# norlab-ulaval/norlab_icp_mapper

Hardware: AMD Instinct MI355X
Metric: ICP iterations/sec, 100k-pt scan vs 1M-pt map (higher is better)
Workload: dtype f32; 1 GPU; single synthetic 100000-pt scan vs 1000000-pt map, point-to-point ICP, KDTreeMatcher knn 1 maxDist 2.0 epsilon 0, TrimmedDist 0.85, fixed 20 iterations per registration; chain=p2p, scene=box+pillars sigma=0.01 seeds 42/43/44 (SURVEY.md 8d), parallelism=scan-sharded x1, map replicated

## Files before the change

### norlab_icp_mapper_amd/csrc/common.h

```cpp
#pragma once

#include <hip/hip_runtime.h>
#include <stdint.h>
#include <math.h>
#include <cstring>
#include <string>
#include <vector>
#include <unordered_map>
#include <mutex>
#include <map>
#include <cstdlib>
#include <shared_mutex>

#include "../../include/icpmi.h"

#define ICPMI_NV 32
#define ICPMI_MAX_OUTLIER 8
#define ICPMI_MAX_SMOOTH 16
#define ICPMI_SEL_BINS 2048
#ifndef ICPMI_S2_COPIES
#define ICPMI_S2_COPIES 8
#endif
#define ICPMI_S2_C0 4096
#define ICPMI_S2_F0 (ICPMI_S2_C0 + ICPMI_S2_COPIES * 256)
#ifndef ICPMI_S2_FCOPIES
#define ICPMI_S2_FCOPIES 1
#endif
#define ICPMI_S2_C1 (ICPMI_S2_F0 + ICPMI_S2_FCOPIES * 65536)
#define ICPMI_S2_F1 (ICPMI_S2_C1 + 256)
#define ICPMI_ACC_COPIES 2
#define ICPMI_ACC_MAX_ADDS 128
#define ICPMI_ACC_PAD 16
#define ICPMI_ACC_U64 (ICPMI_ACC_COPIES * ICPMI_NV * 2 * ICPMI_ACC_PAD)
#define ICPMI_ACC_IDX(copy, i, limb) ((((copy) * ICPMI_NV + (i)) * 2 + (limb)) * ICPMI_ACC_PAD)
#define ICPMI_ACC_FLAG (ICPMI_ACC_IDX(0, 0, 0) + 8)
#define ICPMI_S2_ACC (ICPMI_S2_F1 + 65536)
#define ICPMI_WIN_BINS 7
#ifndef ICPMI_WIN_COPIES
#define ICPMI_WIN_COPIES 8
#endif
#define ICPMI_WIN_PAD 16
#define ICPMI_WIN_HDR (ICPMI_WIN_COPIES * 3 * ICPMI_WIN_PAD)
#define ICPMI_WIN_U64 (ICPMI_WIN_HDR + ICPMI_WIN_PAD)
#define ICPMI_WIN_MAX_COUNT (1ll << 21)
#define ICPMI_S2_WIN (ICPMI_S2_ACC + 2 * ICPMI_ACC_U64)
#define ICPMI_SELHIST_WORDS (ICPMI_S2_WIN + 2 * ICPMI_WIN_U64)
#define ICPMI_S2_FIDX(b) ((((b) & 255u) << 8) | ((b) >> 8))

#define ICPMI_MAX_K 32

#ifdef __HIPCC__
typedef float icpmi_vf4 __attribute__((ext_vector_type(4)));
#ifdef ICPMI_NT_STREAMS
__device__ __forceinline__ float4 ld_stream(const float4* p) { const icpmi_vf4 v = __builtin_nontemporal_load(reinterpret_cast<const icpmi_vf4*>(p)); return make_float4(v.x, v.y, v.z, v.w); }
__device__ __forceinline__ float ld_stream(const float* p) { return __builtin_nontemporal_load(p); }
__device__ __forceinline__ int ld_stream(const int* p) { return __builtin_nontemporal_load(p); }
__device__ __forceinline__ void st_stream(float4* p, float4 v) { icpmi_vf4 w; w.x = v.x; w.y = v.y; w.z = v.z; w.w = v.w; __builtin_nontemporal_store(w, reinterpret_cast<icpmi_vf4*>(p)); }
__device__ __forceinline__ void st_stream(float* p, float v) { __builtin_nontemporal_store(v, p); }
__device__ __forceinline__ void st_stream(int* p, int v) { __builtin_nontemporal_store(v, p); }
#else
template <class T> __device__ __forceinline__ T ld_stream(const T* p) { return *p; }
template <class T> __device__ __forceinline__ void st_stream(T* p, T v) { *p = v; }
#endif

struct WaveRun { bool head; int rank; int len; int head_lane; };
__device__ __forceinline__ WaveRun wave_run(unsigned key, bool valid)
{
    const int lane = threadIdx.x & 63;
    const unsigned prev = (unsigned)__shfl_up((int)key, 1, 64);
    const bool pvalid = __shfl_up((int)valid, 1, 64) != 0;
    const bool head = valid && (lane == 0 || !pvalid || prev != key);
    const unsigned long long heads = __ballot(head);
    const unsigned long long valids = __ballot(valid);
    WaveRun r;
    r.head = head;
    const unsigned long long below = heads & ((lane == 63) ? ~0ull : ((2ull << lane) - 1ull));
    r.head_lane = below ? 63 - __clzll((long long)below) : lane;
    r.rank = lane - r.head_lane;
// ... 747 lines not shown
```

### norlab_icp_mapper_amd/csrc/loop.hip

```cpp
#include "common.h"
#include "solve.h"
#include <cstring>

namespace {

template <int PASS, int MODE = 0>
__global__ __launch_bounds__(256) void sel_hist_kernel(const float* __restrict__ d2, int64_t count,
                                                       const IcpState* __restrict__ st, unsigned* __restrict__ ghist, int nb_scale = 0)
{
    if (st->done) return;
    if (blockIdx.x == 0 && threadIdx.x == 0) nn_stamp_close(const_cast<IcpState*>(st));
    if (MODE != 0 && nb_scale != 0 && st->iter + 1 > nb_scale) return;
    if (MODE == 3 && st->iter != 0) return;
    __shared__ unsigned h[ICPMI_SEL_BINS];
    for (int b = threadIdx.x; b < ICPMI_SEL_BINS; b += 256) h[b] = 0;
    __syncthreads();
    const unsigned prefix = st->sel_prefix;
    const float med = MODE == 2 ? st->robust_med : 0.f;
    for (int64_t i = (int64_t)blockIdx.x * 256 + threadIdx.x; i < count; i += (int64_t)gridDim.x * 256) {
        float v = d2[i];
        if (MODE == 0 || MODE == 3) { if (!(v != INFINITY && v > 0.f)) continue; }
        else {
            if (v == INFINITY) continue;
            if (MODE == 2) v = fabsf(v - med);
// ... 505 lines not shown
                const float rz = fmaf(T[10], az, fmaf(T[6], ay, T[2] * ax));
                ax = rx; ay = ry; az = rz;
            }
            const float4 b = ref_normals[sidx];
            const float dot = fmaf(az, b.z, fmaf(ay, b.y, ax * b.x));
            w *= (dot > cosf(prm)) ? 1.f : 0.f;
        } else if (EXT && type == ICPMI_OUT_GENERICDESCRIPTOR) {
            const int ip = lc.out_iparam[f];
            const float v = (ip & ICPMI_GEN_SOURCE_READING) ? lc.read_scalar[qi] : ref_scalar[orig];
            w *= (ip & ICPMI_GEN_SOFT) ? v : ((ip & ICPMI_GEN_LARGER) ? (v > prm ? 1.f : 0.f) : (v < prm ? 1.f : 0.f));
        } else if (EXT && type == ICPMI_OUT_ROBUST) {
            const int ip = lc.out_iparam[f];
            const int se = (ip >> 4) & 15, fct = ip & 15;
            const float sc = se != ICPMI_SCALE_NONE ? st->robust_scale : 1.f;
            const float res = ((ip >> 8) & 15) == ICPMI_DIST_POINT2PLANE ? plane2 : d2;
            const float kk = se != ICPMI_SCALE_BERG ? prm : (fct == ICPMI_ROB_CAUCHY ? 4.3040f : fct == ICPMI_ROB_TUKEY ? 7.0589f : fct == ICPMI_ROB_HUBER ? 2.0138f : prm);
            const float e2 = res / (sc * sc);
            const float apx = lc.out_param3[f];
            float rw = robust_weight(fct, e2, kk);
            if (apx > 0.f && apx != INFINITY && e2 >= apx * apx) rw = 0.f;
            w *= rw;
        }
    }
    return w;
}

__host__ __device__ __forceinline__ int acc_threads(int k) { return k > 1 ? 1024 : 256; }
__host__ __device__ __forceinline__ int acc_blocks_dev(int64_t count, int cap, int bt = 256)
{
    const int64_t nb = (count + bt - 1) / bt;
    return (int)(nb < 1 ? 1 : (nb > cap ? cap : nb));
}

template <int MIN, bool FUSED, bool EXT, int BT = 256>
__global__ __launch_bounds__(BT) void accumulate_kernel(const float4* __restrict__ reading, BatchArgs ba, int acc_cap, LoopCfg lc,
                                                         IcpState* __restrict__ st, const float4* __restrict__ map,
                                                         const float4* __restrict__ normals,
                                                         const float4* __restrict__ read_normals,
                                                         const int* __restrict__ sidx, const float* __restrict__ d2a,
                                                         unsigned* __restrict__ hists,
                                                         int fused_slot, int is_median, float factor,
                                                         const float4* __restrict__ match_pt, const int* __restrict__ qindex,
                                                         const float* __restrict__ ref_scalar, const float4* __restrict__ pnm)
{
    const int n = ba.n[blockIdx.y];
    const int nbe = acc_blocks_dev((int64_t)n * lc.k, acc_cap, BT);
    if ((int)blockIdx.x >= nbe) return;
    {
        const size_t qo = (size_t)blockIdx.y * (size_t)ba.qstride;
        reading += qo; sidx += qo * lc.k; d2a += qo * lc.k;
        if (match_pt) match_pt += qo;
        if (qindex) qindex += qo;
        if (read_normals) read_normals += qo;
        hists += (size_t)blockIdx.y * ICPMI_SELHIST_WORDS;
        st += blockIdx.y;
    }
    const int64_t count = (int64_t)n * lc.k;
    const int64_t stride = (int64_t)nbe * BT;
    const int64_t gtid = (int64_t)blockIdx.x * BT + threadIdx.x;
#ifdef ICPMI_ACC_STRIDED
    const int64_t estep = stride;
    const int64_t e_first = gtid, e_end = count;
#else
    const int64_t estep = BT;
    const int wgc = (nbe & 7) == 0 ? (int)(blockIdx.x & 7) * (nbe >> 3) + (int)(blockIdx.x >> 3) : (int)blockIdx.x;
    const int64_t per_wg = (count + nbe - 1) / nbe;
    const int64_t e_first = (int64_t)wgc * per_wg + threadIdx.x;
    const int64_t e_end = ((int64_t)wgc + 1) * per_wg < count ? ((int64_t)wgc + 1) * per_wg : count;
#endif
    constexpr int PF = BT > 256 ? 3 : 2;
    float pd2[PF]; int ps[PF]; float4 pr[PF], pq[PF];
#pragma unroll
    for (int u = 0; u < PF; ++u) {
        const int64_t e = e_first + u * estep;
        const bool in = e < e_end;
        pd2[u] = in ? ld_stream(d2a + e) : INFINITY;
        ps[u] = in ? ld_stream(sidx + e) : -1;
        pr[u] = ld_stream(reading + (in ? (int)(e / lc.k) : 0));
        pq[u] = (match_pt && in) ? ld_stream(match_pt + e) : ((pnm && ps[u] >= 0) ? pnm[2 * (size_t)ps[u]] : make_float4(0.f, 0.f, 0.f, 0.f));
    }
    const unsigned cv = (FUSED && threadIdx.x < 256) ? hists[ICPMI_S2_C1 + threadIdx.x] : 0u;
    float4 pn[PF];
#pragma unroll
    for (int u = 0; u < PF; ++u)
        pn[u] = (MIN == ICPMI_MIN_POINT_TO_PLANE && ps[u] >= 0) ? (pnm ? pnm[2 * (size_t)ps[u] + 1] : normals[ps[u]]) : make_float4(0.f, 0.f, 0.f, 0.f);
    if (st->done) return;
    if (blockIdx.x == 0 && threadIdx.x == 0) nn_stamp_close(const_cast<IcpState*>(st));
    float fused_limit = 0.f;
    if (FUSED) {
        __shared__ unsigned shsel[16];
        unsigned bin, rem, total;
        block_find_rank_2tier<1>(cv, hists + ICPMI_S2_F1, false, 0.f, st->sel_rank_l[0], shsel, bin, rem, total);
        const float q = __uint_as_float((st->sel_prefix_l[0] << 16) | bin);
        fused_limit = is_median ? factor * q : q;
        if (blockIdx.x == 0 && threadIdx.x == 0) st->limits[fused_slot] = fused_limit;
        for (int64_t i = gtid; i < ICPMI_S2_COPIES * 256 + ICPMI_S2_FCOPIES * 65536; i += stride) hists[ICPMI_S2_C0 + i] = 0;
        if (lc.k > 1) for (int64_t i = gtid; i < 2 * ICPMI_WIN_U64; i += stride) hists[ICPMI_S2_WIN + i] = 0;
    }
    constexpr int NVAL = MIN == ICPMI_MIN_POINT_TO_PLANE ? 27 : (MIN == ICPMI_MIN_POINT_TO_POINT ? 16 : 0);
    double acc[NVAL > 0 ? NVAL : 1];
#pragma unroll
    for (int i = 0; i < (NVAL > 0 ? NVAL : 1); ++i) acc[i] = 0.0;
    double wsum = 0.0, cnt = 0.0;
    double b2d[3] = {0.0, 0.0, 0.0};
    const float* T = st->T_iter;
    auto pair = [&](int64_t e, float d2, int s, float4 r, float4 qkept, float4 nkept, bool have_n) {
        if (d2 == INFINITY) return;
        const int qi = (int)(e / lc.k);
        float w;
        if (EXT) {
            const float3 pe = xf_point(T, r.x, r.y, r.z, r.w);
            const float4 qe = (match_pt || (pnm && have_n)) ? qkept : (pnm ? pnm[2 * (size_t)s] : map[s]);
            float plane2 = 0.f;
            if (normals) {
                const float4 ne = have_n && MIN == ICPMI_MIN_POINT_TO_PLANE ? nkept : (pnm ? pnm[2 * (size_t)s + 1] : normals[s]);
                const float dx = pe.x - qe.x, dy = pe.y - qe.y, dz = pe.z - qe.z;
                const float dot = dx * ne.x + dy * ne.y + dz * ne.z;
                plane2 = dot * dot;
            }
            w = match_weight<true>(lc, st, d2, T, read_normals, qindex ? qindex[qi] : qi, normals, s, FUSED ? fused_slot : -1, fused_limit,
                                   ref_scalar, __float_as_int(qe.w), plane2);
        } else w = match_weight(lc, st, d2, T, read_normals, qindex ? qindex[qi] : qi, normals, s, FUSED ? fused_slot : -1, fused_limit);
        if (w == 0.f) return;
        wsum += w; cnt += 1.0;
        if (MIN == ICPMI_MIN_IDENTITY) return;
        const float3 p = xf_point(T, r.x, r.y, r.z, r.w);
        const float4 q = (match_pt || (pnm && have_n)) ? qkept : (pnm ? pnm[2 * (size_t)s] : map[s]);
        if (MIN == ICPMI_MIN_POINT_TO_POINT) {
// ... 27 lines not shown
            }
        }
    };
#pragma unroll
    for (int u = 0; u < PF; ++u) pair(e_first + u * estep, pd2[u], ps[u], pr[u], pq[u], pn[u], true);
    for (int64_t e = e_first + PF * estep; e < e_end; e += estep)
        pair(e, d2a[e], sidx[e], reading[(int)(e / lc.k)], match_pt ? match_pt[e] : make_float4(0.f, 0.f, 0.f, 0.f),
             make_float4(0.f, 0.f, 0.f, 0.f), false);
    __shared__ double sh[BT / 64][ICPMI_NV];
    const int lane = threadIdx.x & 63, wv = threadIdx.x >> 6;
    double val[ICPMI_NV];
#pragma unroll
    for (int i = 0; i < ICPMI_NV; ++i) val[i] = i < NVAL ? acc[i < NVAL ? i : 0] : 0.0;
    val[27] = wsum; val[28] = cnt;
    if (EXT) { val[29] = b2d[0]; val[30] = b2d[1]; val[31] = b2d[2]; }
#pragma unroll
    for (int s = 0; s < 5; ++s) {
        const int m = 1 << s;
        const int nkeep = 16 >> s;
        const bool upper = (lane & m) != 0;
#pragma unroll
        for (int i = 0; i < nkeep; ++i) {
            const double send = upper ? val[i] : val[i + nkeep];
            const double keep = upper ? val[i + nkeep] : val[i];
            val[i] = keep + __shfl_xor(send, m, 64);
        }
    }
    val[0] += __shfl_xor(val[0], 32, 64);
    if (lane < 32) {
        const int idx = ((lane & 1) << 4) | ((lane & 2) << 2) | (lane & 4) | ((lane & 8) >> 2) | ((lane & 16) >> 4);
        sh[wv][idx] = val[0];
    }
    __syncthreads();
    if (threadIdx.x < ICPMI_NV) {
        const int i = threadIdx.x;
        double v = 0.0;
        if (i < NVAL || i == 27 || i == 28 || (EXT && i > 28)) {
            v = sh[0][i] + sh[1][i] + sh[2][i] + sh[3][i];
#pragma unroll
            for (int w2 = 4; w2 < BT / 64; ++w2) v += sh[w2][i];
        }
        unsigned long long* acc = reinterpret_cast<unsigned long long*>(hists + ICPMI_S2_ACC);
        if (v != 0.0) {
            if (!(fabs(v) < 0x1p77)) atomicOr(reinterpret_cast<unsigned*>(acc + ICPMI_ACC_FLAG), 1u);
            else {
                const double hi = rint(v * 0x1p-16);
                const double lo = v - hi * 65536.0;
                const long long H = (long long)hi, Lq = __double2ll_rn(lo * 0x1p40);
                const int cp = blockIdx.x & (ICPMI_ACC_COPIES - 1);
                if (H) atomicAdd(acc + ICPMI_ACC_IDX(cp, i, 0), (unsigned long long)H);
                if (Lq) atomicAdd(acc + ICPMI_ACC_IDX(cp, i, 1), (unsigned long long)Lq);
            }
        }
    }
}

__device__ __forceinline__ void mirror_state(const IcpState* st, IcpState* mirror)
{
    const unsigned* src = reinterpret_cast<const unsigned*>(st);
    unsigned* dst = reinterpret_cast<unsigned*>(mirror);
    constexpr int W = (int)(sizeof(IcpState) / sizeof(unsigned));
    for (int i = threadIdx.x; i < W; i += 64) dst[i] = __hip_atomic_load(src + i, __ATOMIC_RELAXED, __HIP_MEMORY_SCOPE_AGENT);
}

__global__ __launch_bounds__(256) void solve_kernel(IcpState* __restrict__ st, unsigned* __restrict__ hists, int clear, LoopCfg lc,
                                                    float* __restrict__ T_step_out, double* __restrict__ sums_out, unsigned* __restrict__ progress,
                                                    IcpState* __restrict__ mirror)
{
    st += blockIdx.x;
    unsigned long long* acc = reinterpret_cast<unsigned long long*>(hists + (size_t)blockIdx.x * ICPMI_SELHIST_WORDS + ICPMI_S2_ACC);
    if (progress) progress += blockIdx.x;
    if (threadIdx.x == 0 && st->hard_count) { st->hard_total += st->hard_count; st->hard_count = 0; }
    if (st->done) {
        if (mirror && threadIdx.x < 64) mirror_state(st, mirror + blockIdx.x);
        if (threadIdx.x == 0) publish_progress(st, progress);
        return;
    }
    solve_body(st, acc, clear != 0, lc, T_step_out, sums_out);
    if (threadIdx.x == 0 && st->done) st->t_done = (unsigned long long)wall_clock64();
    if (mirror) {
        __syncthreads();
        if (threadIdx.x < 64 && __hip_atomic_load(&st->done, __ATOMIC_RELAXED, __HIP_MEMORY_SCOPE_AGENT)) mirror_state(st, mirror + blockIdx.x);
    }
    if (threadIdx.x == 0) publish_progress(st, progress);
}

__global__ __launch_bounds__(256) void centre_kernel(BatchSrc src, BatchArgs ba, float mx, float my, float mz, float4* __restrict__ out)
{
    const int64_t n = ba.n[blockIdx.y];
    const float4* __restrict__ scan = src.p[blockIdx.y];
    out += (size_t)blockIdx.y * (size_t)ba.qstride;
    const int64_t i = (int64_t)blockIdx.x * 256 + threadIdx.x;
    if (i >= n) return;
    const float4 p = scan[i];
    out[i] = make_float4(fmaf(-mx, p.w, p.x), fmaf(-my, p.w, p.y), fmaf(-mz, p.w, p.z), p.w);
// ... 506 lines not shown
    }
    if (slot >= 0) {
        const float quant = lc.out_type[slot] == ICPMI_OUT_MEDIANDIST ? 0.5f : lc.out_param[slot];
        const BatchArgs ba = cur_batch(c, count / lc.k);
        if (!c->nn_builds_hist0)
        {
            int hb0 = (int)std::min<int64_t>((count + 4095) / 4096, 256);
            if (hb0 < 1) hb0 = 1;
            hipLaunchKernelGGL(sel2_hist0_kernel, dim3(hb0, ba.nscan), dim3(256), 0, c->stream, c->d_d2, ba, lc.k, c->d_state, c->d_selhist, quant,
                               c->nn_builds_win ? 1 : 0);
        }
        int hb2 = (int)std::min<int64_t>((count + 511) / 512, 512);
        if (hb2 < 1) hb2 = 1;
        hipLaunchKernelGGL(sel2_scan_hist_kernel, dim3(hb2, ba.nscan), dim3(256), 0, c->stream, c->d_d2, ba, lc.k, c->d_state, c->d_selhist, quant,
                           (c->nn_builds_win && !c->nn_builds_hist0) ? 1 : 0);
        return;
    }
    for (int f = 0; f < lc.n_out; ++f) {
        const int type = lc.out_type[f];
        if (type != ICPMI_OUT_TRIMMEDDIST && type != ICPMI_OUT_MEDIANDIST) continue;
        const int is_med = type == ICPMI_OUT_MEDIANDIST;
        const float quant = is_med ? 0.5f : lc.out_param[f];
        const float factor = lc.out_param[f];
        hipLaunchKernelGGL((sel_hist_kernel<0, 0>), dim3(hb), dim3(256), 0, c->stream, c->d_d2, count, c->d_state, c->d_selhist, 0);
        hipLaunchKernelGGL(sel_scan_kernel<0>, dim3(1), dim3(256), 0, c->stream, c->d_state, c->d_selhist, quant, f, is_med, factor, 0, 0);
        hipLaunchKernelGGL((sel_hist_kernel<1, 0>), dim3(hb), dim3(256), 0, c->stream, c->d_d2, count, c->d_state, c->d_selhist, 0);
        hipLaunchKernelGGL(sel_scan_kernel<1>, dim3(1), dim3(256), 0, c->stream, c->d_state, c->d_selhist, quant, f, is_med, factor, 0, 0);
        hipLaunchKernelGGL((sel_hist_kernel<2, 0>), dim3(hb), dim3(256), 0, c->stream, c->d_d2, count, c->d_state, c->d_selhist, 0);
        hipLaunchKernelGGL(sel_scan_kernel<2>, dim3(1), dim3(256), 0, c->stream, c->d_state, c->d_selhist, quant, f, is_med, factor, 0, 0);
    }
}

template <int MIN, bool FUSED, bool EXT>
static void launch_accumulate_ext(icpmi_ctx* c, int64_t n, const LoopCfg& lc, int nb, int slot);

template <int MIN, bool FUSED>
static void launch_accumulate(icpmi_ctx* c, int64_t n, const LoopCfg& lc, int nb, int slot)
{
    if (lc.ext) launch_accumulate_ext<MIN, FUSED, true>(c, n, lc, nb, slot);
    else launch_accumulate_ext<MIN, FUSED, false>(c, n, lc, nb, slot);
}

template <int MIN, bool FUSED, bool EXT>
static void launch_accumulate_ext(icpmi_ctx* c, int64_t n, const LoopCfg& lc, int nb, int slot)
{
    const float4* rn = lc.has_read_normals ? c->d_read_normals : nullptr;
    const int is_med = slot >= 0 && lc.out_type[slot] == ICPMI_OUT_MEDIANDIST;
    const float factor = slot >= 0 ? lc.out_param[slot] : 0.f;
    const bool sorted = c->nn_out_sorted;
    const BatchArgs ba = cur_batch(c, n);
    if (lc.k > 1) {
        hipLaunchKernelGGL((accumulate_kernel<MIN, FUSED, EXT, 1024>), dim3(nb, ba.nscan), dim3(1024), 0, c->stream, sorted ? c->d_qsorted : c->d_reading, ba, acc_cap(), lc, c->d_state,
                           c->d_map_sorted, c->has_normals ? c->d_normals_sorted : (const float4*)nullptr, rn, c->d_sidx, c->d_d2, c->d_selhist, slot, is_med, factor,
                           (const float4*)nullptr, sorted ? c->d_qindex : (const int*)nullptr, (EXT && c->raw_has_scalar) ? c->d_raw_s : (const float*)nullptr,
                           (MIN == ICPMI_MIN_POINT_TO_PLANE && c->has_normals && c->d_map_pn) ? c->d_map_pn : (const float4*)nullptr);
        return;
    }
    hipLaunchKernelGGL((accumulate_kernel<MIN, FUSED, EXT>), dim3(nb, ba.nscan), dim3(256), 0, c->stream, sorted ? c->d_qsorted : c->d_reading, ba, acc_cap(), lc, c->d_state,
                       c->d_map_sorted, c->has_normals ? c->d_normals_sorted : (const float4*)nullptr, rn, c->d_sidx, c->d_d2, c->d_selhist, slot, is_med, factor,
                       (sorted && lc.k == 1) ? c->d_match_pt : (const float4*)nullptr, sorted ? c->d_qindex : (const int*)nullptr,
                       (EXT && c->raw_has_scalar) ? c->d_raw_s : (const float*)nullptr,
                       (lc.k > 1 && MIN == ICPMI_MIN_POINT_TO_PLANE && c->has_normals && c->d_map_pn) ? c->d_map_pn : (const float4*)nullptr);
}

static void enqueue_accumulate_solve(icpmi_ctx* c, int64_t n, const LoopCfg& lc, float* d_Tstep, double* d_sums)
{
    const int64_t count = n * lc.k;
    const int nb = acc_blocks(count, acc_threads(lc.k));
    const int slot = fused_filter_slot(lc);
    const bool fused = slot >= 0;
    if (lc.minimizer == ICPMI_MIN_POINT_TO_PLANE) {
        if (fused) launch_accumulate<ICPMI_MIN_POINT_TO_PLANE, true>(c, n, lc, nb, slot);
        else launch_accumulate<ICPMI_MIN_POINT_TO_PLANE, false>(c, n, lc, nb, slot);
    } else if (lc.minimizer == ICPMI_MIN_POINT_TO_POINT) {
        if (fused) launch_accumulate<ICPMI_MIN_POINT_TO_POINT, true>(c, n, lc, nb, slot);
        else launch_accumulate<ICPMI_MIN_POINT_TO_POINT, false>(c, n, lc, nb, slot);
    } else {
        if (fused) launch_accumulate<ICPMI_MIN_IDENTITY, true>(c, n, lc, nb, slot);
        else launch_accumulate<ICPMI_MIN_IDENTITY, false>(c, n, lc, nb, slot);
    }
    const BatchArgs ba = cur_batch(c, n);
    hipLaunchKernelGGL(solve_kernel, dim3(ba.nscan), dim3(256), 0, c->stream, c->d_state, c->d_selhist, 1, lc, d_Tstep, d_sums,
                       c->d_progress, ba.nscan == 1 ? c->d_state_mirror : (IcpState*)nullptr);
}

static icpmi_status enqueue_iteration(icpmi_ctx* c, int64_t n, const LoopCfg& lc, hipEvent_t nn0, hipEvent_t nn1)
{
    if (nn0) HIP_TRY(c, hipEventRecord(nn0, c->stream));
    c->nn_hist0 = fused_filter_slot(lc) >= 0 ? c->d_selhist : nullptr;
    c->nn_builds_hist0 = false;
    c->nn_builds_win = false;
    c->nn_match_pt = lc.k == 1 ? c->d_match_pt : nullptr;
    c->nn_sorted_k = lc.k > 1;
    c->nn_out_sorted = false;
    icpmi_status s = nn_launch_k(c, c->d_reading, n, c->d_state->T_iter, lc, 1, c->d_sidx, c->d_d2, c->d_state);
    c->nn_sorted_k = false;
    if (s != ICPMI_OK) return s;
    if (nn1) HIP_TRY(c, hipEventRecord(nn1, c->stream));
    enqueue_selection(c, lc, n * lc.k);
    enqueue_accumulate_solve(c, n, lc, nullptr, nullptr);
    HIP_TRY(c, hipGetLastError());
    return ICPMI_OK;
}

static void fill_stats(const IcpState* hs, const LoopCfg& lc, int64_t n, icpmi_stats* stats, bool with_dbg = true)
{
    if (!stats) return;
    stats->iterations = hs->iter;
    stats->stop_reason = hs->stop_reason;
    stats->pairs = hs->pairs;
    const double denom = (double)lc.k * (double)n;
    stats->point_used_ratio = denom > 0 ? (float)hs->pairs / (float)denom : 0.f;
    stats->weighted_point_used_ratio = denom > 0 ? (float)(hs->wsum / denom) : 0.f;
    stats->trimmed_limit = -1.f;
    for (int f = 0; f < lc.n_out; ++f)
        if (lc.out_type[f] == ICPMI_OUT_TRIMMEDDIST || lc.out_type[f] == ICPMI_OUT_MEDIANDIST || lc.out_type[f] == ICPMI_OUT_VARTRIMMEDDIST) stats->trimmed_limit = hs->limits[f];
// ... 495 lines not shown
```

### norlab_icp_mapper_amd/csrc/solve.h

```cpp
#pragma once
#include "common.h"

namespace {

__device__ void mat4_mul_dev(const float* A, const float* B, float* C)
{
    float R[16];
#pragma unroll
    for (int j = 0; j < 4; ++j)
#pragma unroll
        for (int i = 0; i < 4; ++i) {
            float s = A[i] * B[4 * j];
#pragma unroll
            for (int kk = 1; kk < 4; ++kk) s = fmaf(A[4 * kk + i], B[4 * j + kk], s);
            R[4 * j + i] = s;
        }
#pragma unroll
    for (int i = 0; i < 16; ++i) C[i] = R[i];
}

__device__ void jacobi_eig(int n, const double* Ain, double* w, double* Q)
{
    __shared__ double A[36];
    for (int i = 0; i < n * n; ++i) A[i] = Ain[i];
// ... 336 lines not shown
        s = fmaf(nrm * z, ps, nrm);
        float pc = fmaf(z, -2.75573192e-07f, 2.48015873e-05f);
        pc = fmaf(z, pc, -1.38888889e-03f);
        pc = fmaf(z, pc, 4.16666667e-02f);
        pc = fmaf(z, pc, -0.5f);
        c = fmaf(z, pc, 1.f);
    } else { s = (float)sin((double)nrm); c = (float)cos((double)nrm); }
    const float sx = s * ax, sy = s * ay, sz = s * az;
    const float cx = (1.f - c) * ax, cy = (1.f - c) * ay, cz = (1.f - c) * az;
    float tmp;
    tmp = cx * ay; T[4 * 1 + 0] = tmp - sz; T[4 * 0 + 1] = tmp + sz;
    tmp = cx * az; T[4 * 2 + 0] = tmp + sy; T[4 * 0 + 2] = tmp - sy;
    tmp = cy * az; T[4 * 2 + 1] = tmp - sx; T[4 * 1 + 2] = tmp + sx;
    T[0] = cx * ax + c; T[5] = cy * ay + c; T[10] = cz * az + c;
}

__device__ double quat_angdist(const double* a, const double* b)
{
    const double w = a[0] * b[0] + a[1] * b[1] + a[2] * b[2] + a[3] * b[3];
    const double x = -a[0] * b[1] + a[1] * b[0] - a[2] * b[3] + a[3] * b[2];
    const double y = -a[0] * b[2] + a[1] * b[3] + a[2] * b[0] - a[3] * b[1];
    const double z = -a[0] * b[3] - a[1] * b[2] + a[2] * b[1] + a[3] * b[0];
    return 2.0 * atan2(sqrt(x * x + y * y + z * z), fabs(w));
}

__device__ __forceinline__ unsigned pair_sum_mask(const LoopCfg& lc)
{
    const unsigned nval = lc.minimizer == ICPMI_MIN_POINT_TO_PLANE ? 27u : (lc.minimizer == ICPMI_MIN_POINT_TO_POINT ? 16u : 0u);
    unsigned m = (nval ? ((1u << nval) - 1u) : 0u) | (1u << 27) | (1u << 28);
    if (lc.force_2d) m |= 7u << 29;
    return m;
}

__device__ __forceinline__ void read_pair_sums(unsigned long long* __restrict__ acc, double* __restrict__ tot , bool clear, bool* nonfinite,
                                               unsigned mask = 0xffffffffu)
{
    __shared__ long long ph[ICPMI_ACC_COPIES][ICPMI_NV], pl[ICPMI_ACC_COPIES][ICPMI_NV];
    __shared__ unsigned s_flag;
    const int t = threadIdx.x;
    if (t < ICPMI_ACC_COPIES * ICPMI_NV) {
        const int i = t & (ICPMI_NV - 1), cp = t >> 5;
        unsigned long long a = 0ull, b = 0ull;
        if ((mask >> i) & 1u) { a = acc[ICPMI_ACC_IDX(cp, i, 0)]; b = acc[ICPMI_ACC_IDX(cp, i, 1)]; }
        ph[cp][i] = (long long)a; pl[cp][i] = (long long)b;
        if (clear) { if (a) acc[ICPMI_ACC_IDX(cp, i, 0)] = 0ull; if (b) acc[ICPMI_ACC_IDX(cp, i, 1)] = 0ull; }
    }
    if (t == ICPMI_ACC_COPIES * ICPMI_NV) {
        unsigned* fl = reinterpret_cast<unsigned*>(acc + ICPMI_ACC_FLAG);
        s_flag = *fl;
        if (clear && s_flag) *fl = 0u;
    }
    __syncthreads();
    if (t < ICPMI_NV) {
        long long H = 0, Lq = 0;
#pragma unroll
        for (int cp = 0; cp < ICPMI_ACC_COPIES; ++cp) { H += ph[cp][t]; Lq += pl[cp][t]; }
        tot[t] = (double)H * 65536.0 + (double)Lq * 0x1p-40;
    }
    __syncthreads();
    *nonfinite = s_flag != 0u;
}

__device__ void solve_serial(IcpState* st, const double* tot, const LoopCfg& lc, float* T_step_out)
{
    const long long tsolve0 = clock64();

    const double wsum = tot[27];
    const long long P = (long long)(tot[28] + 0.5);
    st->pairs = P;
    st->wsum = wsum;
    if (P == 0) { st->error = ICPMI_ERR_NO_POINT_TO_MINIMIZE; st->done = 1; return; }

    float Ts[16];
    for (int i = 0; i < 16; ++i) Ts[i] = (i % 5 == 0) ? 1.f : 0.f;
    if (lc.minimizer == ICPMI_MIN_POINT_TO_POINT) {
        const double iw = 1.0 / wsum;
        const double mpd[3] = {tot[1] * iw, tot[2] * iw, tot[3] * iw}, mqd[3] = {tot[4] * iw, tot[5] * iw, tot[6] * iw};
        __shared__ float H[9];
        for (int c = 0; c < 3; ++c)
            for (int r = 0; r < 3; ++r) H[3 * c + r] = (float)(tot[7 + 3 * c + r] - mqd[r] * tot[1 + c]);
        __shared__ float R[9];
        if (lc.is_2d) {
            const float a = H[0] + H[4], b2 = H[1] - H[3];
            const float r = sqrtf(a * a + b2 * b2);
            float cs = 1.f, sn = 0.f;
            if (r > 0.f) { cs = a / r; sn = b2 / r; }
            for (int i = 0; i < 9; ++i) R[i] = 0.f;
            R[0] = cs; R[1] = sn; R[3] = -sn; R[4] = cs; R[8] = 1.f;
        } else rotation_from_H(H, R);
        const float mp[3] = {(float)mpd[0], (float)mpd[1], (float)mpd[2]};
        const float mq[3] = {(float)mqd[0], (float)mqd[1], (float)mqd[2]};
        for (int c = 0; c < 3; ++c) for (int r = 0; r < 3; ++r) Ts[4 * c + r] = R[3 * c + r];
        for (int r = 0; r < 3; ++r) Ts[12 + r] = mq[r] - (R[r] * mp[0] + R[3 + r] * mp[1] + R[6 + r] * mp[2]);
    } else if (lc.minimizer == ICPMI_MIN_POINT_TO_PLANE) {
        __shared__ float A[36], b[6], x[6];
        auto fill_Ab = [&]() {
            int idx = 0;
            for (int a = 0; a < 6; ++a)
                for (int bb = a; bb < 6; ++bb) { const float v = (float)tot[idx++]; A[6 * a + bb] = v; A[6 * bb + a] = v; }
            for (int a = 0; a < 6; ++a) b[a] = (float)tot[21 + a];
        };
        if (lc.force_2d || lc.force_4dof) fill_Ab();
        if (lc.force_2d) {
            __shared__ float A3[9], b3[3], x3[3];
            for (int c = 0; c < 3; ++c) { b3[c] = (float)tot[29 + c]; for (int r = 0; r < 3; ++r) A3[3 * c + r] = A[6 * (2 + c) + (2 + r)]; }
            solve_spd<3>(A3, b3, x3);
            x[0] = 0.f; x[1] = 0.f; x[2] = x3[0]; x[3] = x3[1]; x[4] = x3[2]; x[5] = 0.f;
        } else if (lc.force_4dof) {
            __shared__ float A4[16], b4[4], x4[4];
            for (int c = 0; c < 4; ++c) { b4[c] = b[2 + c]; for (int r = 0; r < 4; ++r) A4[4 * c + r] = A[6 * (2 + c) + (2 + r)]; }
            solve_spd<4>(A4, b4, x4);
            x[0] = 0.f; x[1] = 0.f; x[2] = x4[0]; x[3] = x4[1]; x[4] = x4[2]; x[5] = x4[3];
        } else {
            auto tri = [](int r, int c) { return r * 6 - r * (r - 1) / 2 + (c - r); };
            const bool ok = chol_solve<6>([&](int i, int j) { return (float)tot[tri(j < i ? j : i, j < i ? i : j)]; },
                                          [&](int i) { return (float)tot[21 + i]; }, x);
            if (!ok) { fill_Ab(); solve_min_norm(6, A, b, x); }
        }
        angle_axis_T(x, Ts);
        Ts[12] = x[3]; Ts[13] = x[4]; Ts[14] = x[5];
    }
    const long long tsolve1 = clock64();
    for (int i = 0; i < 16; ++i)
        if (Ts[i] != Ts[i]) { st->error = ICPMI_ERR_NAN; st->done = 1; return; }
    if (T_step_out) for (int i = 0; i < 16; ++i) T_step_out[i] = Ts[i];

    float Ti[16];
    mat4_mul_dev(Ts, st->T_iter, Ti);
    for (int i = 0; i < 16; ++i) st->T_prev[i] = st->T_iter[i];
    for (int i = 0; i < 16; ++i) st->T_iter[i] = Ti[i];
    st->iter += 1;

    const long long tsolve2 = clock64();
    bool iterate = true;
    int reason = ICPMI_STOP_NONE;
    st->counter += 1;
    if (st->counter >= lc.max_iter) { iterate = false; reason = ICPMI_STOP_COUNTER; }
    if (lc.use_diff) {
        const int SL = lc.smooth;
        const int RING = ICPMI_MAX_SMOOTH + 1;
        const int slot = st->hist_n % RING;
        quat_from_T(Ti, st->hq + 4 * slot);
        for (int r = 0; r < 3; ++r) st->ht[3 * slot + r] = Ti[12 + r];
        st->hist_n += 1;
        const int hn = st->hist_n;
        {
            const int a = (hn - 1) % RING, bq = (hn - 2) % RING;
            st->hrot[a] = fabs(quat_angdist(st->hq + 4 * a, st->hq + 4 * bq));
            const double dx = st->ht[3 * a] - st->ht[3 * bq], dy = st->ht[3 * a + 1] - st->ht[3 * bq + 1],
                         dz = st->ht[3 * a + 2] - st->ht[3 * bq + 2];
            st->htr[a] = sqrt(dx * dx + dy * dy + dz * dz);
        }
        if (hn > SL) {
            double rot = 0, tr = 0;
            for (int i = hn - 1; i >= hn - SL; --i) { rot += st->hrot[i % RING]; tr += st->htr[i % RING]; }
            rot /= SL; tr /= SL;
            if (rot != rot || tr != tr) { st->error = ICPMI_ERR_NAN; st->done = 1; return; }
            if (rot < (double)lc.min_rot && tr < (double)lc.min_trans) {
                if (iterate) reason = ICPMI_STOP_DIFFERENTIAL;
                iterate = false;
            }
        }
    }
    if (lc.use_bound) {
        __shared__ double q[4];
        quat_from_T(Ti, q);
        const double rot = fabs(quat_angdist(q, st->init_q));
        const double nt = sqrt((double)Ti[12] * Ti[12] + (double)Ti[13] * Ti[13] + (double)Ti[14] * Ti[14]);
        if (rot > (double)lc.max_rot || nt > (double)lc.max_trans) { st->error = ICPMI_ERR_BOUND; st->done = 1; return; }
    }
    if (!iterate) { st->done = 1; st->stop_reason = reason; }
    const long long tsolve3 = clock64();
#ifndef ICPMI_NN_TIMING
    st->dbg[20] += (unsigned long long)(tsolve3 - tsolve0);
    st->dbg[21] += 1;
    st->dbg[22] += (unsigned long long)(tsolve1 - tsolve0);
    st->dbg[23] += (unsigned long long)(tsolve3 - tsolve2);
#else
    (void)tsolve1; (void)tsolve2; (void)tsolve3;
#endif
}

__device__ void solve_body(IcpState* __restrict__ st, unsigned long long* __restrict__ acc, bool clear, const LoopCfg& lc,
                           float* __restrict__ T_step_out, double* __restrict__ sums_out)
{
    __shared__ double tot[ICPMI_NV];
    const int t = threadIdx.x;
    bool nonfinite = false;
    read_pair_sums(acc, tot, clear, &nonfinite, pair_sum_mask(lc));
    if (t < ICPMI_NV && sums_out) sums_out[t] = tot[t];
    if (nonfinite) { if (t == 0) { st->error = ICPMI_ERR_NAN; st->done = 1; } return; }
    if (t == 0) solve_serial(st, tot, lc, T_step_out);
}

__device__ __forceinline__ void publish_progress(const IcpState* st, unsigned* progress)
{
    if (!progress) return;
    const unsigned v = ((unsigned)(st->done != 0) << 31) | ((st->seq & 0x7ffffu) << 12) | ((unsigned)st->iter & 0xfffu);
    __hip_atomic_store(progress, v, __ATOMIC_RELEASE, __HIP_MEMORY_SCOPE_SYSTEM);
}
struct ProgressWord { bool mine, done; int iter; };
static inline ProgressWord decode_progress(unsigned v, unsigned seq) { return {((v >> 12) & 0x7ffffu) == seq, (v >> 31) != 0, (int)(v & 0xfffu)}; }


}
```

Measured before the change: 23750 iterations/s.

## Fuse ICP solve into accumulate kernel via last-block ticket

Removes the separate solve_kernel launch per ICP iteration. The last accumulate block to finish, detected with an atomic ticket counter, now runs the solve in place. That block stages IcpState in shared memory, overlaps those loads with the pair-sum loads, and writes back only the words that changed. The old path is kept behind a macro. This saves one kernel launch and dependency per iteration, at the cost of an extra atomic plus waitcnt in every block and a serial tail inside one block.

Result: no change. 23520 iterations/s (-1.0%).

```diff
diff --git a/norlab_icp_mapper_amd/csrc/common.h b/norlab_icp_mapper_amd/csrc/common.h
--- a/norlab_icp_mapper_amd/csrc/common.h
+++ b/norlab_icp_mapper_amd/csrc/common.h
@@ -43,7 +43,11 @@
 #define ICPMI_WIN_HDR (ICPMI_WIN_COPIES * 3 * ICPMI_WIN_PAD)
 #define ICPMI_WIN_U64 (ICPMI_WIN_HDR + ICPMI_WIN_PAD)
 #define ICPMI_WIN_MAX_COUNT (1ll << 21)
-#define ICPMI_S2_WIN (ICPMI_S2_ACC + 2 * ICPMI_ACC_U64)
+#define ICPMI_S2_TICKET (ICPMI_S2_ACC + 2 * ICPMI_ACC_U64)
+#ifndef ICPMI_SOLVE_TICKET
+#define ICPMI_SOLVE_LAUNCH 1
+#endif
+#define ICPMI_S2_WIN (ICPMI_S2_TICKET + 32)
 #define ICPMI_SELHIST_WORDS (ICPMI_S2_WIN + 2 * ICPMI_WIN_U64)
 #define ICPMI_S2_FIDX(b) ((((b) & 255u) << 8) | ((b) >> 8))
 
diff --git a/norlab_icp_mapper_amd/csrc/loop.hip b/norlab_icp_mapper_amd/csrc/loop.hip
--- a/norlab_icp_mapper_amd/csrc/loop.hip
+++ b/norlab_icp_mapper_amd/csrc/loop.hip
@@ -561,6 +561,63 @@
     return (int)(nb < 1 ? 1 : (nb > cap ? cap : nb));
 }
 
+__device__ __forceinline__ void mirror_state(const IcpState* st, IcpState* mirror)
+{
+    const unsigned* src = reinterpret_cast<const unsigned*>(st);
+    unsigned* dst = reinterpret_cast<unsigned*>(mirror);
+    constexpr int W = (int)(sizeof(IcpState) / sizeof(unsigned));
+    for (int i = threadIdx.x; i < W; i += 64) dst[i] = __hip_atomic_load(src + i, __ATOMIC_RELAXED, __HIP_MEMORY_SCOPE_AGENT);
+}
+
+__device__ __forceinline__ void solve_tail_done(IcpState* st, unsigned* progress, IcpState* mirror)
+{
+    if (threadIdx.x == 0 && st->hard_count) { st->hard_total += st->hard_count; st->hard_count = 0; }
+    if (mirror && threadIdx.x < 64) mirror_state(st, mirror);
+    if (threadIdx.x == 0) publish_progress(st, progress);
+}
+
+template <int MIN, int BT>
+__device__ __forceinline__ void solve_tail(IcpState* __restrict__ st, unsigned* __restrict__ hists, const LoopCfg& lc, float* __restrict__ T_step_out,
+                                           double* __restrict__ sums_out, unsigned* __restrict__ progress, IcpState* __restrict__ mirror)
+{
+    constexpr int W = (int)(sizeof(IcpState) / sizeof(unsigned));
+    constexpr int PER = (W + BT - 1) / BT;
+    static_assert(sizeof(IcpState) % sizeof(unsigned) == 0 && BT >= 256, "state staged word by word, by the threads solve_body needs");
+    __shared__ IcpState s_st;
+    unsigned* const sw = reinterpret_cast<unsigned*>(&s_st);
+    unsigned* const gw = reinterpret_cast<unsigned*>(st);
+    unsigned w0[PER];
+    unsigned long long* acc = reinterpret_cast<unsigned long long*>(hists + ICPMI_S2_ACC);
+    solve_body<MIN>(&s_st, acc, true, lc, T_step_out, sums_out, [&] {
+#pragma unroll
+        for (int u = 0; u < PER; ++u) {
+            const int i = (int)threadIdx.x + u * BT;
+            w0[u] = __hip_atomic_load(gw + (i < W ? i : 0), __ATOMIC_RELAXED, __HIP_MEMORY_SCOPE_AGENT);
+        }
+#pragma unroll
+        for (int u = 0; u < PER; ++u) {
+            const int i = (int)threadIdx.x + u * BT;
+            if (i < W) sw[i] = w0[u];
+        }
+    });
+    if (threadIdx.x == 0) {
+        __hip_atomic_store(hists + ICPMI_S2_TICKET, 0u, __ATOMIC_RELAXED, __HIP_MEMORY_SCOPE_AGENT);
+        if (s_st.hard_count) { s_st.hard_total += s_st.hard_count; s_st.hard_count = 0; }
+        if (s_st.done) s_st.t_done = (unsigned long long)wall_clock64();
+    }
+    __syncthreads();
+#pragma unroll
+    for (int u = 0; u < PER; ++u) {
+        const int i = (int)threadIdx.x + u * BT;
+        if (i < W && sw[i] != w0[u]) gw[i] = sw[i];
+    }
+    if (mirror && threadIdx.x < 64 && s_st.done) {
+        unsigned* dst = reinterpret_cast<unsigned*>(mirror);
+        for (int i = threadIdx.x; i < W; i += 64) dst[i] = sw[i];
+    }
+    if (threadIdx.x == 0) publish_progress(&s_st, progress);
+}
+
 template <int MIN, bool FUSED, bool EXT, int BT = 256>
 __global__ __launch_bounds__(BT) void accumulate_kernel(const float4* __restrict__ reading, BatchArgs ba, int acc_cap, LoopCfg lc,
                                                          IcpState* __restrict__ st, const float4* __restrict__ map,
@@ -570,7 +627,9 @@
                                                          unsigned* __restrict__ hists,
                                                          int fused_slot, int is_median, float factor,
                                                          const float4* __restrict__ match_pt, const int* __restrict__ qindex,
-                                                         const float* __restrict__ ref_scalar, const float4* __restrict__ pnm)
+                                                         const float* __restrict__ ref_scalar, const float4* __restrict__ pnm,
+                                                         float* __restrict__ T_step_out, double* __restrict__ sums_out,
+                                                         unsigned* __restrict__ progress, IcpState* __restrict__ mirror)
 {
     const int n = ba.n[blockIdx.y];
     const int nbe = acc_blocks_dev((int64_t)n * lc.k, acc_cap, BT);
@@ -583,6 +642,7 @@
         if (read_normals) read_normals += qo;
         hists += (size_t)blockIdx.y * ICPMI_SELHIST_WORDS;
         st += blockIdx.y;
+        if (progress) progress += blockIdx.y;
     }
     const int64_t count = (int64_t)n * lc.k;
     const int64_t stride = (int64_t)nbe * BT;
@@ -613,8 +673,18 @@
 #pragma unroll
     for (int u = 0; u < PF; ++u)
         pn[u] = (MIN == ICPMI_MIN_POINT_TO_PLANE && ps[u] >= 0) ? (pnm ? pnm[2 * (size_t)ps[u] + 1] : normals[ps[u]]) : make_float4(0.f, 0.f, 0.f, 0.f);
+#ifdef ICPMI_SOLVE_LAUNCH
     if (st->done) return;
     if (blockIdx.x == 0 && threadIdx.x == 0) nn_stamp_close(const_cast<IcpState*>(st));
+#else
+    if (st->done) {
+        if (blockIdx.x == 0) solve_tail_done(st, progress, mirror);
+        return;
+    }
+    unsigned long long nn_begin = 0ull, nn_sum = 0ull, nn_close = 0ull;
+    unsigned nn_cnt = 0u;
+    if (blockIdx.x == 0 && threadIdx.x == 0) { nn_begin = st->t_nn_begin; nn_sum = st->t_nn_sum; nn_cnt = st->nn_count; nn_close = (unsigned long long)wall_clock64(); }
+#endif
     float fused_limit = 0.f;
     if (FUSED) {
         __shared__ unsigned shsel[16];
@@ -622,7 +692,9 @@
         block_find_rank_2tier<1>(cv, hists + ICPMI_S2_F1, false, 0.f, st->sel_rank_l[0], shsel, bin, rem, total);
         const float q = __uint_as_float((st->sel_prefix_l[0] << 16) | bin);
         fused_limit = is_median ? factor * q : q;
+#ifdef ICPMI_SOLVE_LAUNCH
         if (blockIdx.x == 0 && threadIdx.x == 0) st->limits[fused_slot] = fused_limit;
+#endif
         for (int64_t i = gtid; i < ICPMI_S2_COPIES * 256 + ICPMI_S2_FCOPIES * 65536; i += stride) hists[ICPMI_S2_C0 + i] = 0;
         if (lc.k > 1) for (int64_t i = gtid; i < 2 * ICPMI_WIN_U64; i += stride) hists[ICPMI_S2_WIN + i] = 0;
     }
@@ -716,6 +788,8 @@
         sh[wv][idx] = val[0];
     }
     __syncthreads();
+    unsigned long long ret_h = 0ull, ret_l = 0ull;
+    unsigned ret_f = 0u;
     if (threadIdx.x < ICPMI_NV) {
         const int i = threadIdx.x;
         double v = 0.0;
@@ -726,25 +800,37 @@
         }
         unsigned long long* acc = reinterpret_cast<unsigned long long*>(hists + ICPMI_S2_ACC);
         if (v != 0.0) {
-            if (!(fabs(v) < 0x1p77)) atomicOr(reinterpret_cast<unsigned*>(acc + ICPMI_ACC_FLAG), 1u);
+            if (!(fabs(v) < 0x1p77)) ret_f = atomicOr(reinterpret_cast<unsigned*>(acc + ICPMI_ACC_FLAG), 1u);
             else {
                 const double hi = rint(v * 0x1p-16);
                 const double lo = v - hi * 65536.0;
                 const long long H = (long long)hi, Lq = __double2ll_rn(lo * 0x1p40);
                 const int cp = blockIdx.x & (ICPMI_ACC_COPIES - 1);
-                if (H) atomicAdd(acc + ICPMI_ACC_IDX(cp, i, 0), (unsigned long long)H);
-                if (Lq) atomicAdd(acc + ICPMI_ACC_IDX(cp, i, 1), (unsigned long long)Lq);
+                if (H) ret_h = atomicAdd(acc + ICPMI_ACC_IDX(cp, i, 0), (unsigned long long)H);
+                if (Lq) ret_l = atomicAdd(acc + ICPMI_ACC_IDX(cp, i, 1), (unsigned long long)Lq);
             }
         }
     }
-}
-
-__device__ __forceinline__ void mirror_state(const IcpState* st, IcpState* mirror)
-{
-    const unsigned* src = reinterpret_cast<const unsigned*>(st);
-    unsigned* dst = reinterpret_cast<unsigned*>(mirror);
-    constexpr int W = (int)(sizeof(IcpState) / sizeof(unsigned));
-    for (int i = threadIdx.x; i < W; i += 64) dst[i] = __hip_atomic_load(src + i, __ATOMIC_RELAXED, __HIP_MEMORY_SCOPE_AGENT);
+#ifndef ICPMI_SOLVE_LAUNCH
+    __shared__ unsigned s_last;
+    unsigned long long ret_s = 0ull, ret_b = 0ull;
+    unsigned ret_c = 0u, ret_m = 0u;
+    if (blockIdx.x == 0 && threadIdx.x == 0) {
+        if (nn_begin) {
+            ret_s = __hip_atomic_exchange(&st->t_nn_sum, nn_sum + (nn_close - nn_begin), __ATOMIC_RELAXED, __HIP_MEMORY_SCOPE_AGENT);
+            ret_c = __hip_atomic_exchange(&st->nn_count, nn_cnt + 1u, __ATOMIC_RELAXED, __HIP_MEMORY_SCOPE_AGENT);
+            ret_b = __hip_atomic_exchange(&st->t_nn_begin, 0ull, __ATOMIC_RELAXED, __HIP_MEMORY_SCOPE_AGENT);
+        }
+        if (FUSED) ret_m = __hip_atomic_exchange(reinterpret_cast<unsigned*>(&st->limits[fused_slot]), __float_as_uint(fused_limit), __ATOMIC_RELAXED, __HIP_MEMORY_SCOPE_AGENT);
+    }
+    asm volatile("" :: "v"(ret_h), "v"(ret_l), "v"(ret_f), "v"(ret_s), "v"(ret_c), "v"(ret_b), "v"(ret_m) : "memory");
+    asm volatile("s_waitcnt vmcnt(0)" ::: "memory");
+    if (threadIdx.x == 0)
+        s_last = __hip_atomic_fetch_add(hists + ICPMI_S2_TICKET, 1u, __ATOMIC_RELAXED, __HIP_MEMORY_SCOPE_AGENT) == (unsigned)(nbe - 1) ? 1u : 0u;
+    __syncthreads();
+    if (!s_last) return;
+    solve_tail<MIN, BT>(st, hists, lc, T_step_out, sums_out, progress, mirror);
+#endif
 }
 
 __global__ __launch_bounds__(256) void solve_kernel(IcpState* __restrict__ st, unsigned* __restrict__ hists, int clear, LoopCfg lc,
@@ -1317,35 +1403,38 @@
 }
 
 template <int MIN, bool FUSED, bool EXT>
-static void launch_accumulate_ext(icpmi_ctx* c, int64_t n, const LoopCfg& lc, int nb, int slot);
+static void launch_accumulate_ext(icpmi_ctx* c, int64_t n, const LoopCfg& lc, int nb, int slot, float* d_Tstep, double* d_sums);
 
 template <int MIN, bool FUSED>
-static void launch_accumulate(icpmi_ctx* c, int64_t n, const LoopCfg& lc, int nb, int slot)
-{
-    if (lc.ext) launch_accumulate_ext<MIN, FUSED, true>(c, n, lc, nb, slot);
-    else launch_accumulate_ext<MIN, FUSED, false>(c, n, lc, nb, slot);
+static void launch_accumulate(icpmi_ctx* c, int64_t n, const LoopCfg& lc, int nb, int slot, float* d_Tstep, double* d_sums)
+{
+    if (lc.ext) launch_accumulate_ext<MIN, FUSED, true>(c, n, lc, nb, slot, d_Tstep, d_sums);
+    else launch_accumulate_ext<MIN, FUSED, false>(c, n, lc, nb, slot, d_Tstep, d_sums);
 }
 
 template <int MIN, bool FUSED, bool EXT>
-static void launch_accumulate_ext(icpmi_ctx* c, int64_t n, const LoopCfg& lc, int nb, int slot)
+static void launch_accumulate_ext(icpmi_ctx* c, int64_t n, const LoopCfg& lc, int nb, int slot, float* d_Tstep, double* d_sums)
 {
     const float4* rn = lc.has_read_normals ? c->d_read_normals : nullptr;
     const int is_med = slot >= 0 && lc.out_type[slot] == ICPMI_OUT_MEDIANDIST;
     const float factor = slot >= 0 ? lc.out_param[slot] : 0.f;
     const bool sorted = c->nn_out_sorted;
     const BatchArgs ba = cur_batch(c, n);
+    IcpState* mirror = ba.nscan == 1 ? c->d_state_mirror : (IcpState*)nullptr;
     if (lc.k > 1) {
         hipLaunchKernelGGL((accumulate_kernel<MIN, FUSED, EXT, 1024>), dim3(nb, ba.nscan), dim3(1024), 0, c->stream, sorted ? c->d_qsorted : c->d_reading, ba, acc_cap(), lc, c->d_state,
                            c->d_map_sorted, c->has_normals ? c->d_normals_sorted : (const float4*)nullptr, rn, c->d_sidx, c->d_d2, c->d_selhist, slot, is_med, factor,
                            (const float4*)nullptr, sorted ? c->d_qindex : (const int*)nullptr, (EXT && c->raw_has_scalar) ? c->d_raw_s : (const float*)nullptr,
-                           (MIN == ICPMI_MIN_POINT_TO_PLANE && c->has_normals && c->d_map_pn) ? c->d_map_pn : (const float4*)nullptr);
+                           (MIN == ICPMI_MIN_POINT_TO_PLANE && c->has_normals && c->d_map_pn) ? c->d_map_pn : (const float4*)nullptr,
+                           d_Tstep, d_sums, c->d_progress, mirror);
         return;
     }
     hipLaunchKernelGGL((accumulate_kernel<MIN, FUSED, EXT>), dim3(nb, ba.nscan), dim3(256), 0, c->stream, sorted ? c->d_qsorted : c->d_reading, ba, acc_cap(), lc, c->d_state,
                        c->d_map_sorted, c->has_normals ? c->d_normals_sorted : (const float4*)nullptr, rn, c->d_sidx, c->d_d2, c->d_selhist, slot, is_med, factor,
                        (sorted && lc.k == 1) ? c->d_match_pt : (const float4*)nullptr, sorted ? c->d_qindex : (const int*)nullptr,
                        (EXT && c->raw_has_scalar) ? c->d_raw_s : (const float*)nullptr,
-                       (lc.k > 1 && MIN == ICPMI_MIN_POINT_TO_PLANE && c->has_normals && c->d_map_pn) ? c->d_map_pn : (const float4*)nullptr);
+                       (lc.k > 1 && MIN == ICPMI_MIN_POINT_TO_PLANE && c->has_normals && c->d_map_pn) ? c->d_map_pn : (const float4*)nullptr,
+                       d_Tstep, d_sums, c->d_progress, mirror);
 }
 
 static void enqueue_accumulate_solve(icpmi_ctx* c, int64_t n, const LoopCfg& lc, float* d_Tstep, double* d_sums)
@@ -1355,18 +1444,20 @@
     const int slot = fused_filter_slot(lc);
     const bool fused = slot >= 0;
     if (lc.minimizer == ICPMI_MIN_POINT_TO_PLANE) {
-        if (fused) launch_accumulate<ICPMI_MIN_POINT_TO_PLANE, true>(c, n, lc, nb, slot);
-        else launch_accumulate<ICPMI_MIN_POINT_TO_PLANE, false>(c, n, lc, nb, slot);
+        if (fused) launch_accumulate<ICPMI_MIN_POINT_TO_PLANE, true>(c, n, lc, nb, slot, d_Tstep, d_sums);
+        else launch_accumulate<ICPMI_MIN_POINT_TO_PLANE, false>(c, n, lc, nb, slot, d_Tstep, d_sums);
     } else if (lc.minimizer == ICPMI_MIN_POINT_TO_POINT) {
-        if (fused) launch_accumulate<ICPMI_MIN_POINT_TO_POINT, true>(c, n, lc, nb, slot);
-        else launch_accumulate<ICPMI_MIN_POINT_TO_POINT, false>(c, n, lc, nb, slot);
+        if (fused) launch_accumulate<ICPMI_MIN_POINT_TO_POINT, true>(c, n, lc, nb, slot, d_Tstep, d_sums);
+        else launch_accumulate<ICPMI_MIN_POINT_TO_POINT, false>(c, n, lc, nb, slot, d_Tstep, d_sums);
     } else {
-        if (fused) launch_accumulate<ICPMI_MIN_IDENTITY, true>(c, n, lc, nb, slot);
-        else launch_accumulate<ICPMI_MIN_IDENTITY, false>(c, n, lc, nb, slot);
-    }
+        if (fused) launch_accumulate<ICPMI_MIN_IDENTITY, true>(c, n, lc, nb, slot, d_Tstep, d_sums);
+        else launch_accumulate<ICPMI_MIN_IDENTITY, false>(c, n, lc, nb, slot, d_Tstep, d_sums);
+    }
+#ifdef ICPMI_SOLVE_LAUNCH
     const BatchArgs ba = cur_batch(c, n);
     hipLaunchKernelGGL(solve_kernel, dim3(ba.nscan), dim3(256), 0, c->stream, c->d_state, c->d_selhist, 1, lc, d_Tstep, d_sums,
                        c->d_progress, ba.nscan == 1 ? c->d_state_mirror : (IcpState*)nullptr);
+#endif
 }
 
 static icpmi_status enqueue_iteration(icpmi_ctx* c, int64_t n, const LoopCfg& lc, hipEvent_t nn0, hipEvent_t nn1)
diff --git a/norlab_icp_mapper_amd/csrc/solve.h b/norlab_icp_mapper_amd/csrc/solve.h
--- a/norlab_icp_mapper_amd/csrc/solve.h
+++ b/norlab_icp_mapper_amd/csrc/solve.h
@@ -392,23 +392,37 @@
     return m;
 }
 
-__device__ __forceinline__ void read_pair_sums(unsigned long long* __restrict__ acc, double* __restrict__ tot , bool clear, bool* nonfinite,
-                                               unsigned mask = 0xffffffffu)
+struct PairSumLoads { unsigned long long a, b; unsigned flag; };
+__device__ __forceinline__ PairSumLoads pair_sums_issue(const unsigned long long* __restrict__ acc, unsigned mask)
+{
+    PairSumLoads L = {0ull, 0ull, 0u};
+    const int t = threadIdx.x;
+    if (t < ICPMI_ACC_COPIES * ICPMI_NV) {
+        const int i = t & (ICPMI_NV - 1), cp = t >> 5;
+        if ((mask >> i) & 1u) {
+            L.a = __hip_atomic_load(acc + ICPMI_ACC_IDX(cp, i, 0), __ATOMIC_RELAXED, __HIP_MEMORY_SCOPE_AGENT);
+            L.b = __hip_atomic_load(acc + ICPMI_ACC_IDX(cp, i, 1), __ATOMIC_RELAXED, __HIP_MEMORY_SCOPE_AGENT);
+        }
+    }
+    if (t == ICPMI_ACC_COPIES * ICPMI_NV)
+        L.flag = __hip_atomic_load(reinterpret_cast<const unsigned*>(acc + ICPMI_ACC_FLAG), __ATOMIC_RELAXED, __HIP_MEMORY_SCOPE_AGENT);
+    return L;
+}
+
+__device__ __forceinline__ void pair_sums_finish(unsigned long long* __restrict__ acc, const PairSumLoads& L, double* __restrict__ tot ,
+                                                 bool clear, bool* nonfinite)
 {
     __shared__ long long ph[ICPMI_ACC_COPIES][ICPMI_NV], pl[ICPMI_ACC_COPIES][ICPMI_NV];
     __shared__ unsigned s_flag;
     const int t = threadIdx.x;
     if (t < ICPMI_ACC_COPIES * ICPMI_NV) {
         const int i = t & (ICPMI_NV - 1), cp = t >> 5;
-        unsigned long long a = 0ull, b = 0ull;
-        if ((mask >> i) & 1u) { a = acc[ICPMI_ACC_IDX(cp, i, 0)]; b = acc[ICPMI_ACC_IDX(cp, i, 1)]; }
-        ph[cp][i] = (long long)a; pl[cp][i] = (long long)b;
-        if (clear) { if (a) acc[ICPMI_ACC_IDX(cp, i, 0)] = 0ull; if (b) acc[ICPMI_ACC_IDX(cp, i, 1)] = 0ull; }
+        ph[cp][i] = (long long)L.a; pl[cp][i] = (long long)L.b;
+        if (clear) { if (L.a) acc[ICPMI_ACC_IDX(cp, i, 0)] = 0ull; if (L.b) acc[ICPMI_ACC_IDX(cp, i, 1)] = 0ull; }
     }
     if (t == ICPMI_ACC_COPIES * ICPMI_NV) {
-        unsigned* fl = reinterpret_cast<unsigned*>(acc + ICPMI_ACC_FLAG);
-        s_flag = *fl;
-        if (clear && s_flag) *fl = 0u;
+        s_flag = L.flag;
+        if (clear && L.flag) *reinterpret_cast<unsigned*>(acc + ICPMI_ACC_FLAG) = 0u;
     }
     __syncthreads();
     if (t < ICPMI_NV) {
@@ -421,9 +435,11 @@
     *nonfinite = s_flag != 0u;
 }
 
+template <int MINT = -1>
 __device__ void solve_serial(IcpState* st, const double* tot, const LoopCfg& lc, float* T_step_out)
 {
     const long long tsolve0 = clock64();
+    const int minimizer = MINT >= 0 ? MINT : lc.minimizer;
 
     const double wsum = tot[27];
     const long long P = (long long)(tot[28] + 0.5);
@@ -433,7 +449,7 @@
 
     float Ts[16];
     for (int i = 0; i < 16; ++i) Ts[i] = (i % 5 == 0) ? 1.f : 0.f;
-    if (lc.minimizer == ICPMI_MIN_POINT_TO_POINT) {
+    if (minimizer == ICPMI_MIN_POINT_TO_POINT) {
         const double iw = 1.0 / wsum;
         const double mpd[3] = {tot[1] * iw, tot[2] * iw, tot[3] * iw}, mqd[3] = {tot[4] * iw, tot[5] * iw, tot[6] * iw};
         __shared__ float H[9];
@@ -452,7 +468,7 @@
         const float mq[3] = {(float)mqd[0], (float)mqd[1], (float)mqd[2]};
         for (int c = 0; c < 3; ++c) for (int r = 0; r < 3; ++r) Ts[4 * c + r] = R[3 * c + r];
         for (int r = 0; r < 3; ++r) Ts[12 + r] = mq[r] - (R[r] * mp[0] + R[3 + r] * mp[1] + R[6 + r] * mp[2]);
-    } else if (lc.minimizer == ICPMI_MIN_POINT_TO_PLANE) {
+    } else if (minimizer == ICPMI_MIN_POINT_TO_PLANE) {
         __shared__ float A[36], b[6], x[6];
         auto fill_Ab = [&]() {
             int idx = 0;
@@ -494,13 +510,15 @@
     const long long tsolve2 = clock64();
     bool iterate = true;
     int reason = ICPMI_STOP_NONE;
+    __shared__ float Tq[16];
+    if (lc.use_diff || lc.use_bound) for (int i = 0; i < 16; ++i) Tq[i] = Ti[i];
     st->counter += 1;
     if (st->counter >= lc.max_iter) { iterate = false; reason = ICPMI_STOP_COUNTER; }
     if (lc.use_diff) {
         const int SL = lc.smooth;
         const int RING = ICPMI_MAX_SMOOTH + 1;
         const int slot = st->hist_n % RING;
-        quat_from_T(Ti, st->hq + 4 * slot);
+        quat_from_T(Tq, st->hq + 4 * slot);
         for (int r = 0; r < 3; ++r) st->ht[3 * slot + r] = Ti[12 + r];
         st->hist_n += 1;
         const int hn = st->hist_n;
@@ -524,7 +542,7 @@
     }
     if (lc.use_bound) {
         __shared__ double q[4];
-        quat_from_T(Ti, q);
+        quat_from_T(Tq, q);
         const double rot = fabs(quat_angdist(q, st->init_q));
         const double nt = sqrt((double)Ti[12] * Ti[12] + (double)Ti[13] * Ti[13] + (double)Ti[14] * Ti[14]);
         if (rot > (double)lc.max_rot || nt > (double)lc.max_trans) { st->error = ICPMI_ERR_BOUND; st->done = 1; return; }
@@ -541,16 +559,24 @@
 #endif
 }
 
-__device__ void solve_body(IcpState* __restrict__ st, unsigned long long* __restrict__ acc, bool clear, const LoopCfg& lc,
-                           float* __restrict__ T_step_out, double* __restrict__ sums_out)
+template <int MINT = -1, class Stage>
+__device__ __forceinline__ void solve_body(IcpState* st, unsigned long long* __restrict__ acc, bool clear, const LoopCfg& lc,
+                                           float* __restrict__ T_step_out, double* __restrict__ sums_out, Stage stage)
 {
     __shared__ double tot[ICPMI_NV];
     const int t = threadIdx.x;
     bool nonfinite = false;
-    read_pair_sums(acc, tot, clear, &nonfinite, pair_sum_mask(lc));
+    const PairSumLoads L = pair_sums_issue(acc, pair_sum_mask(lc));
+    stage();
+    pair_sums_finish(acc, L, tot, clear, &nonfinite);
     if (t < ICPMI_NV && sums_out) sums_out[t] = tot[t];
     if (nonfinite) { if (t == 0) { st->error = ICPMI_ERR_NAN; st->done = 1; } return; }
-    if (t == 0) solve_serial(st, tot, lc, T_step_out);
+    if (t == 0) solve_serial<MINT>(st, tot, lc, T_step_out);
+}
+__device__ void solve_body(IcpState* __restrict__ st, unsigned long long* __restrict__ acc, bool clear, const LoopCfg& lc,
+                           float* __restrict__ T_step_out, double* __restrict__ sums_out)
+{
+    solve_body(st, acc, clear, lc, T_step_out, sums_out, [] {});
 }
 
 __device__ __forceinline__ void publish_progress(const IcpState* st, unsigned* progress)
```
